# phlash/java-sdr

Hardware: AMD Instinct MI355X
Metric: IQ Msamples/s through FFT+FIR+BPSK demod, 2048-pt frames (higher is better)
Workload: dtype f64

## Files before the change

### java-sdr_amd/binding.py

```python
import ctypes as C
import os
import re

import numpy as np

HERE = os.path.dirname(os.path.abspath(__file__))
ROOT = os.path.dirname(HERE)
_SO = os.environ.get("JSDR_LIB") or os.path.join(HERE, "libjsdr_hip.so")


class JsdrError(RuntimeError):
    pass


def library_path():
    return _SO


def _declared_symbols():
    hdr = open(os.path.join(ROOT, "include", "jsdr_hip.h")).read()
    hdr = re.sub(r"/\*.*?\*/", " ", hdr, flags=re.S)
    return sorted(set(re.findall(r"\b(jsdr_[a-z0-9_]+)\s*\(", hdr)))


# ... 805 lines not shown
                                                        tu if tunings else None, ff, up, C.c_int64(self.max_batch)),
                   "jsdr_bpsk_create_live_channels")
            return
        if do_fft is not None:
            ff = (C.c_int * max(self.nchannels, 1))(*[int(v) for v in do_fft])
            _check(lib().jsdr_bpsk_create_mode_channels(C.byref(self.h), rate, self.samples, ninputs, self.nchannels,
                                                        tu if tunings else None, ff, up, C.c_int64(self.max_batch)),
                   "jsdr_bpsk_create_mode_channels")
            return
        _check(lib().jsdr_bpsk_create_channels(C.byref(self.h), rate, self.samples, ninputs, self.nchannels, tu if tunings else None,
                                               up, C.c_int64(self.max_batch)), "jsdr_bpsk_create_channels")

    def acq_last_launch(self):
        a, b = C.c_int64(), C.c_int64()
        _check(lib().jsdr_bpsk_acq_last_launch(self.h, C.byref(a), C.byref(b)), "jsdr_bpsk_acq_last_launch")
        return a.value, b.value

    def stream(self, inp, ch):
        return inp * self.nchannels + ch

    def channel_info(self):
        a, b = C.c_int(), C.c_int()
        _check(lib().jsdr_bpsk_channel_info(self.h, C.byref(a), C.byref(b)), "jsdr_bpsk_channel_info")
        return a.value, b.value

    def batch_i16(self, raw_dev, input_stride_i16, nsamples, ic=0, qc=0, stream=None):
        super().batch_i16(raw_dev, input_stride_i16, nsamples, ic, qc, stream)

    def batch_f32(self, iq_dev, input_stride_f32, nsamples, stream=None):
        super().batch_f32(iq_dev, input_stride_f32, nsamples, stream)

    def set_channel_tuning(self, channel, tuning_hz):
        _check(lib().jsdr_bpsk_set_channel_tuning(self.h, int(channel), C.c_double(tuning_hz)), "jsdr_bpsk_set_channel_tuning")

    def set_channel_mode(self, channel, do_fft, do_up):
        _check(lib().jsdr_bpsk_set_channel_mode(self.h, int(channel), int(do_fft), int(do_up)), "jsdr_bpsk_set_channel_mode")

    def channel_control(self, channel):
        t, f, u = C.c_double(), C.c_int(), C.c_int()
        _check(lib().jsdr_bpsk_get_channel_control(self.h, int(channel), C.byref(t), C.byref(f), C.byref(u)),
               "jsdr_bpsk_get_channel_control")
        return t.value, f.value, u.value

    def counters(self, inp=0, ch=0):
        return super().counters(self.stream(inp, ch))

    def bits(self, inp=0, ch=0):
        return super().bits(self.stream(inp, ch))

    def fec_results(self, inp=0, ch=0):
        return super().fec_results(self.stream(inp, ch))

    def decoded(self, inp=0, ch=0):
        return super().decoded(self.stream(inp, ch))

    def trace(self, inp=0, ch=0):
        return super().trace(self.stream(inp, ch))

    def state(self, inp=0, ch=0):
        return super().state(self.stream(inp, ch))


class Group:

    def __init__(self, ndev, total_streams, max_batch_samples, devices=None, rate=96000, frame=2048, tuning=12000, do_fft=0,
                 do_up=0, gather_copy=False, with_psd=False):
        self.h = C.c_void_p()
        self.ndev = ndev
        devs = (C.c_int * ndev)(*devices) if devices is not None else None
        flags = (1 if gather_copy else 0) | (2 if with_psd else 0)
        _check(lib().jsdr_group_create(C.byref(self.h), ndev, devs, rate, frame, tuning, do_fft, do_up, total_streams,
                                       C.c_int64(max_batch_samples), flags), "jsdr_group_create")
        n, s, sb, v = C.c_int(), C.c_int(), C.c_int64(), C.c_int()
        _check(lib().jsdr_group_info(self.h, C.byref(n), C.byref(s), C.byref(sb), C.byref(v)), "jsdr_group_info")
        self.streams_per_device, self.slot_bytes, self.rccl_version = s.value, sb.value, v.value
        self.total_streams = total_streams

    def device(self, index):
        d, dem, fft = C.c_int(), C.c_void_p(), C.c_void_p()
        _check(lib().jsdr_group_device(self.h, index, C.byref(d), C.byref(dem), C.byref(fft)), "jsdr_group_device")
        view = Bpsk.__new__(Bpsk)
        view.h, view.nstreams, view.borrowed = dem, self.streams_per_device, True
        return d.value, view

    def batch_i16(self, raw_devs, stride_i16, nsamples, ic=0, qc=0, psd_devs=None):
        raws = (C.c_void_p * self.ndev)(*[_addr(r) for r in raw_devs])
        psds = (C.c_void_p * self.ndev)(*[_addr(p) for p in psd_devs]) if psd_devs is not None else None
        _check(lib().jsdr_group_batch_i16(self.h, raws, C.c_int64(stride_i16), C.c_int64(nsamples), ic, qc, psds),
               "jsdr_group_batch_i16")

    def sync(self):
        _check(lib().jsdr_group_sync(self.h), "jsdr_group_sync")

    def set_tuning(self, tuning_hz):
        _check(lib().jsdr_group_set_tuning(self.h, C.c_double(tuning_hz)), "jsdr_group_set_tuning")

    def set_mode(self, do_fft, do_up):
        _check(lib().jsdr_group_set_mode(self.h, int(do_fft), int(do_up)), "jsdr_group_set_mode")

    def read_slot(self, index, stream):
        out = np.empty(self.slot_bytes, np.uint8)
        _check(lib().jsdr_group_read_slot(self.h, index, stream, _addr(out)), "jsdr_group_read_slot")
        return out

    def gathered(self, index):
        p, nb = C.c_void_p(), C.c_int64()
        self.sync()
        _check(lib().jsdr_group_gathered(self.h, index, C.byref(p), C.byref(nb)), "jsdr_group_gathered")
        dev, _ = self.device(index)
        out = np.empty(nb.value, np.uint8)
        _check(lib().jsdr_set_device(dev), "jsdr_set_device")
        _check(lib().jsdr_memcpy_d2h(_addr(out), p, C.c_size_t(nb.value)), "jsdr_memcpy_d2h")
        return out.reshape(self.total_streams, self.slot_bytes)

    def __del__(self):
        try:
            lib().jsdr_group_destroy(self.h)
        except Exception:
            pass


def unpack_slot(slot, info):
    hdr = np.frombuffer(slot[:64], np.int32)
    nb, nt = int(hdr[0]), int(hdr[1])
    bits = np.frombuffer(slot[info["bits_offset"]:info["bits_offset"] + nb], np.int8)
    fec = []
    for t in range(nt):
        o = info["fec_offset"] + t * 264
        rc, bi = np.frombuffer(slot[o:o + 8], np.int32)
        fec.append((int(rc), int(bi), np.frombuffer(slot[o + 8:o + 264], np.uint8)))
    names = ["nbits", "nfec"] + COUNTER_NAMES[:9]
    return dict(header=dict(zip(names, (int(v) for v in hdr[:11]))), bits=bits, fec=fec)


def demod_scope_layout(n, width):
    out = [np.zeros(max(int(width), 0), np.int32) for _ in range(4)]
    _check(lib().jsdr_demod_scope_layout(int(n), int(width), *[_addr(a) if a.size else None for a in out], int(width)),
           "jsdr_demod_scope_layout")
    return tuple(out)


class Demod:

    def __init__(self, rate=96000, n=2048, nstreams=1, max_batch_samples=None):
        self.rate, self.n, self.S = rate, n, nstreams
        self.max_batch = max_batch_samples or n
        self.h = C.c_void_p()
        _check(lib().jsdr_demod_create(C.byref(self.h), rate, n, nstreams, C.c_int64(self.max_batch)), "jsdr_demod_create")

    def configure(self, mode, dofir=0, dodwn=0, doagc=0):
        _check(lib().jsdr_demod_configure(self.h, mode, dofir, dodwn, doagc), "jsdr_demod_configure")

    def weights(self, flo, fhi):
        w = np.empty(21, np.float32)
        phi = C.c_float()
        _check(lib().jsdr_demod_weights(self.h, flo, fhi, _addr(w), C.byref(phi)), "jsdr_demod_weights")
        return w, np.float32(phi.value)

    def batch_i16(self, raw_dev, stride_i16, nsamples, audio_dev, audio_stride_i16, ic=0, qc=0, stream=None):
        _check(lib().jsdr_demod_batch_i16(self.h, _addr(raw_dev), C.c_int64(stride_i16), C.c_int64(nsamples), ic, qc,
                                          _addr(audio_dev), C.c_int64(audio_stride_i16), C.c_void_p(stream)),
               "jsdr_demod_batch_i16")

    def batch_f32(self, iq_dev, stride_f32, nsamples, audio_dev, audio_stride_i16, stream=None):
        _check(lib().jsdr_demod_batch_f32(self.h, _addr(iq_dev), C.c_int64(stride_f32), C.c_int64(nsamples),
                                          _addr(audio_dev), C.c_int64(audio_stride_i16), C.c_void_p(stream)),
               "jsdr_demod_batch_f32")

    def batch_host_i16(self, raw, nsamples, ic=0, qc=0):
        raw = np.ascontiguousarray(raw, np.int16).reshape(self.S, 2 * nsamples)
        d_in = DeviceBuffer.from_host(raw)
        d_out = DeviceBuffer(raw.nbytes)
        self.batch_i16(d_in, 2 * nsamples, nsamples, d_out, 2 * nsamples, ic, qc)
        return d_out.to_host(np.int16).reshape(self.S, 2 * nsamples)

    def receive(self, buf):
        buf = np.ascontiguousarray(buf, np.float32)
        assert buf.size == 2 * self.n
        out = np.empty(2 * self.n, np.int16)
        _check(lib().jsdr_demod_receive_f32(self.h, _addr(buf), _addr(out)), "jsdr_demod_receive_f32")
        return out

    def frame_stats(self, stream=0):
        mx, av = C.c_float(), C.c_float()
        _check(lib().jsdr_demod_frame_stats(self.h, stream, C.byref(mx), C.byref(av)), "jsdr_demod_frame_stats")
        return np.float32(mx.value), np.float32(av.value)

    def state(self):
        car, phi = C.c_float(), C.c_float()
        _check(lib().jsdr_demod_state(self.h, C.byref(car), C.byref(phi)), "jsdr_demod_state")
        return np.float32(car.value), np.float32(phi.value)

    def scope_i16(self, raw_dev, stride_i16, nsamples, audio_dev, audio_stride_i16, width, height, trace_dev=None, spec_dev=None,
                  dbg_dev=None, ic=0, qc=0, stream=None):
        _check(lib().jsdr_demod_scope_i16(self.h, _addr(raw_dev), C.c_int64(stride_i16), C.c_int64(nsamples), int(ic), int(qc),
                                          _addr(audio_dev), C.c_int64(audio_stride_i16), int(width), int(height), _addr(trace_dev),
                                          _addr(spec_dev), _addr(dbg_dev), C.c_void_p(stream)), "jsdr_demod_scope_i16")

    def scope_f32(self, iq_dev, stride_f32, nsamples, audio_dev, audio_stride_i16, width, height, trace_dev=None, spec_dev=None,
                  dbg_dev=None, stream=None):
        _check(lib().jsdr_demod_scope_f32(self.h, _addr(iq_dev), C.c_int64(stride_f32), C.c_int64(nsamples), _addr(audio_dev),
                                          C.c_int64(audio_stride_i16), int(width), int(height), _addr(trace_dev), _addr(spec_dev),
                                          _addr(dbg_dev), C.c_void_p(stream)), "jsdr_demod_scope_f32")

    def scope_chunk(self, frames):
        _check(lib().jsdr_demod_scope_chunk(self.h, int(frames)), "jsdr_demod_scope_chunk")

    def scope_kernel(self):
        return lib().jsdr_demod_scope_kernel(self.h).decode()

    def profile_enable(self, on):
        _check(lib().jsdr_demod_profile_enable(self.h, int(on)), "jsdr_demod_profile_enable")

    def profile_read(self):
        k = lib().jsdr_demod_profile_count()
        ms = np.zeros(k, np.float64)
        cnt = np.zeros(k, np.int32)
        _check(lib().jsdr_demod_profile_read(self.h, _addr(ms), _addr(cnt)), "jsdr_demod_profile_read")
        return {lib().jsdr_demod_profile_name(i).decode(): (float(ms[i]), int(cnt[i])) for i in range(k)}

    def __del__(self):
        try:
            lib().jsdr_demod_destroy(self.h)
        except Exception:
            pass


class DemodChannels(Demod):

    def __init__(self, rate=96000, n=2048, ninputs=1, nchannels=1, max_batch_samples=None):
        self.rate, self.n, self.ninputs, self.nchannels = rate, n, ninputs, nchannels
        self.S = ninputs * nchannels
        self.max_batch = max_batch_samples or n
        self.h = C.c_void_p()
        _check(lib().jsdr_demod_create_channels(C.byref(self.h), rate, n, ninputs, nchannels, C.c_int64(self.max_batch)),
               "jsdr_demod_create_channels")

    def stream(self, inp, ch):
        return inp * self.nchannels + ch

    def channel_info(self):
        a, b = C.c_int(), C.c_int()
        _check(lib().jsdr_demod_channel_info(self.h, C.byref(a), C.byref(b)), "jsdr_demod_channel_info")
        return a.value, b.value

    def configure_channel(self, channel, mode, dofir=0, dodwn=0, doagc=0):
        _check(lib().jsdr_demod_configure_channel(self.h, int(channel), int(mode), int(dofir), int(dodwn), int(doagc)),
               "jsdr_demod_configure_channel")

    def channel_weights(self, channel, flo, fhi):
        w = np.empty(21, np.float32)
        phi = C.c_float()
        _check(lib().jsdr_demod_channel_weights(self.h, int(channel), int(flo), int(fhi), _addr(w), C.byref(phi)),
               "jsdr_demod_channel_weights")
        return w, np.float32(phi.value)

    def channel_control(self, channel):
        v = [C.c_int() for _ in range(6)]
        _check(lib().jsdr_demod_get_channel(self.h, int(channel), *[C.byref(x) for x in v]), "jsdr_demod_get_channel")
        return tuple(x.value for x in v)

    def channel_state(self, channel):
        car, phi = C.c_float(), C.c_float()
        _check(lib().jsdr_demod_channel_state(self.h, int(channel), C.byref(car), C.byref(phi)), "jsdr_demod_channel_state")
        return np.float32(car.value), np.float32(phi.value)

    def batch_i16(self, raw_dev, input_stride_i16, nsamples, audio_dev, audio_stride_i16, ic=0, qc=0, stream=None):
        super().batch_i16(raw_dev, input_stride_i16, nsamples, audio_dev, audio_stride_i16, ic, qc, stream)

    def batch_f32(self, iq_dev, input_stride_f32, nsamples, audio_dev, audio_stride_i16, stream=None):
        super().batch_f32(iq_dev, input_stride_f32, nsamples, audio_dev, audio_stride_i16, stream)

    def batch_host_i16(self, raw, nsamples, ic=0, qc=0):
        raw = np.ascontiguousarray(raw, np.int16).reshape(self.ninputs, 2 * nsamples)
        d_in = DeviceBuffer.from_host(raw)
        d_out = DeviceBuffer(self.S * 2 * nsamples * 2)
        self.batch_i16(d_in, 2 * nsamples, nsamples, d_out, 2 * nsamples, ic, qc)
        return d_out.to_host(np.int16).reshape(self.ninputs, self.nchannels, 2 * nsamples)

    def receive(self, buf):
        buf = np.ascontiguousarray(buf, np.float32)
        assert buf.size == 2 * self.n
        out = np.empty(self.nchannels * 2 * self.n, np.int16)
        _check(lib().jsdr_demod_receive_f32(self.h, _addr(buf), _addr(out)), "jsdr_demod_receive_f32")
        return out.reshape(self.nchannels, 2 * self.n)


class RecordingInfo(C.Structure):
    _fields_ = [("format", C.c_int), ("encoding", C.c_int), ("channels", C.c_int), ("rate", C.c_int),
                ("bits", C.c_int), ("frames", C.c_int64), ("data_offset", C.c_int64)]


def waterfall_lines(psd, n, width, peak_rgb=0x00FFFF):
    psd = np.ascontiguousarray(psd, np.float32).reshape(-1, n + 2)
    d_in = DeviceBuffer.from_host(psd)
    d_out = DeviceBuffer(4 * psd.shape[0] * width)
    _check(lib().jsdr_waterfall_lines(_addr(d_in), C.c_int64(psd.shape[0]), n, width, C.c_uint32(peak_rgb),
                                      _addr(d_out), None), "jsdr_waterfall_lines")
    return d_out.to_host(np.uint32).reshape(psd.shape[0], width)


def waterfall_lines_dev(psd_dev, nframes, n, width, pix_dev, peak_rgb=0x00FFFF, stream=None):
    _check(lib().jsdr_waterfall_lines(_addr(psd_dev), C.c_int64(nframes), n, width, C.c_uint32(peak_rgb),
                                      _addr(pix_dev), stream), "jsdr_waterfall_lines")


def recording_probe(path, raw_channels=2):
    info = RecordingInfo()
    _check(lib().jsdr_recording_probe(os.fsencode(path), raw_channels, C.byref(info)), "jsdr_recording_probe")
    return info


def recordings_load(paths, channels, rate, first_frame, nframes, raw_dev, stream_stride_i16):
    arr = (C.c_char_p * len(paths))(*[os.fsencode(p) for p in paths])
    got = (C.c_int64 * len(paths))()
    _check(lib().jsdr_recordings_load(arr, len(paths), channels, rate, C.c_int64(first_frame), C.c_int64(nframes),
                                      _addr(raw_dev), C.c_int64(stream_stride_i16), got, None), "jsdr_recordings_load")
    return list(got)


def synth_mix64(z):
    m = 0xFFFFFFFFFFFFFFFF
    z = (z + 0x9E3779B97F4A7C15) & m
    z = ((z ^ (z >> 30)) * 0xBF58476D1CE4E5B9) & m
    z = ((z ^ (z >> 27)) * 0x94D049BB133111EB) & m
    return z ^ (z >> 31)


def synth_carrier_tables(amp):
    a = 2.0 * np.pi * np.arange(1024, dtype=np.float64) / 1024.0
    return np.rint(amp * np.cos(a)).astype(np.int16), np.rint(amp * np.sin(a)).astype(np.int16)


def synth_phase_inc_u32(freq_hz, rate):
    return int(round(freq_hz / rate * 2 ** 32)) & 0xFFFFFFFF


def synth_payloads(seed, stream0, nstreams, nframes, out_dev=None, stream=None):
    own = out_dev is None
    if own:
        out_dev = DeviceBuffer(nstreams * nframes * 256)
    _check(lib().jsdr_synth_payloads(C.c_uint64(seed), stream0, nstreams, nframes, _addr(out_dev), C.c_void_p(stream)),
           "jsdr_synth_payloads")
    return out_dev


def synth_diffsign(sym_dev, nsym, nstreams, dsign_dev, stream=None):
    _check(lib().jsdr_synth_diffsign(_addr(sym_dev), C.c_int64(nsym), nstreams, _addr(dsign_dev), C.c_void_p(stream)),
           "jsdr_synth_diffsign")


def synth_dbpsk(out_dev, stride_i16, nstreams, n0, n, dsign_dev, nsym, sps, phase0, phase_inc, cos_dev, sin_dev,
                noise_gain, keys_dev, stream=None):
    _check(lib().jsdr_synth_dbpsk(_addr(out_dev), C.c_int64(stride_i16), nstreams, C.c_int64(n0), C.c_int64(n),
                                  _addr(dsign_dev), C.c_int64(nsym), sps, C.c_uint32(phase0), C.c_uint32(phase_inc),
                                  _addr(cos_dev), _addr(sin_dev), noise_gain, _addr(keys_dev), C.c_void_p(stream)),
           "jsdr_synth_dbpsk")


def synth_tones(out_dev, frame0, nframes, n, cos_dev, noise_gain, key, stream=None):
    _check(lib().jsdr_synth_tones(_addr(out_dev), C.c_int64(frame0), C.c_int64(nframes), n, _addr(cos_dev), noise_gain,
                                  C.c_uint64(key), C.c_void_p(stream)), "jsdr_synth_tones")
```

### java-sdr_amd/csrc/fft_block_body.h

```cpp
    extern __shared__ __align__(16) unsigned char smem[];
    constexpr int FE = lds_frame_elems(N);
    constexpr int TWN = TWG ? 0 : tw_total(R0, R1, R2, R3);
    float2 *tw_own = reinterpret_cast<float2 *>(smem);
    float2 *bufs = tw_own + TWN;
    float *red_val = reinterpret_cast<float *>(bufs + (size_t)FPB * FE);
    int *red_idx = reinterpret_cast<int *>(red_val + FPB * ((T + 63) / 64));
    const float2 *tw_lds = TWG ? a.tw : tw_own;
#ifdef JSDR_X_WGCLK
    const unsigned long long wgclk0 = __builtin_amdgcn_s_memrealtime();
    unsigned long long wgclk_n = 0;
#endif

    const int tid_b = threadIdx.x;
    if constexpr (!TWG) {
        for (int i = tid_b; i < TWN; i += T * FPB) tw_own[i] = a.tw[i];
        __syncthreads();
    }

    const int fib = tid_b / T;
    const int tid = tid_b - fib * T;
    float2 *buf = bufs + (size_t)fib * FE;
    const long long ngroups = (a.nframes + FPB - 1) / FPB;
    auto frame_of = [&](long long g) {
        long long f = g * FPB + fib;
        return f < a.nframes ? f : a.nframes - 1;
    };
    typename RawPoint<IN>::type raw[R0];
    if ((long long)blockIdx.x < ngroups) fft_fetch<N, T, IN, R0>(a, frame_of(blockIdx.x), tid, raw);
    for (long long g = blockIdx.x; g < ngroups; g += gridDim.x) {
        const long long gn = g + gridDim.x;
        fft_frame<N, T, IN, OUT, R0, R1, R2, R3>(a, frame_of(g), frame_of(gn < ngroups ? gn : g), tid, buf, tw_lds, red_val,
                                                 red_idx, fib, raw);
        __syncthreads();
#ifdef JSDR_X_WGCLK
        wgclk_n++;
#endif
    }
#ifdef JSDR_X_WGCLK
    if (tid_b == 0 && blockIdx.x < WGCLK_WGS) {
        unsigned long long *c = g_fft_wgclk[a.wgclk_slot][blockIdx.x];
        c[0] = wgclk0;
        c[1] = __builtin_amdgcn_s_memrealtime();
        c[2] = wgclk_n;
    }
#endif
```

### java-sdr_amd/csrc/fft_common.h

```cpp
#pragma once
#include "common.h"
#include <type_traits>
#include <utility>
#include <vector>

namespace jsdr {

constexpr double cx_pi = 3.14159265358979323846264338327950288;

constexpr double cx_sin_small(double x)
{
    double x2 = x * x, term = x, sum = x;
    for (int i = 1; i < 12; i++) {
        term *= -x2 / ((2 * i) * (2 * i + 1));
        sum += term;
    }
    return sum;
}
constexpr double cx_cos_small(double x)
{
    double x2 = x * x, term = 1.0, sum = 1.0;
    for (int i = 1; i < 12; i++) {
        term *= -x2 / ((2 * i - 1) * (2 * i));
        sum += term;
    }
    return sum;
}
constexpr double cx_cos_turn(int j, int len)
{
    j %= len;
    if (8 * j <= len) return cx_cos_small(2 * cx_pi * j / len);
    if (8 * j <= 3 * len) return -cx_sin_small(2 * cx_pi * (j - 0.25 * len) / len);
    if (8 * j <= 5 * len) return -cx_cos_small(2 * cx_pi * (j - 0.5 * len) / len);
    if (8 * j <= 7 * len) return cx_sin_small(2 * cx_pi * (j - 0.75 * len) / len);
    return cx_cos_small(2 * cx_pi * (j - len) / len);
}
constexpr double cx_sin_turn(int j, int len) { return cx_cos_turn(4 * j + 3 * len, 4 * len); }

typedef float v2f __attribute__((ext_vector_type(2)));
__device__ __forceinline__ v2f to_v(float2 a) { return (v2f){a.x, a.y}; }
__device__ __forceinline__ float2 from_v(v2f v) { return make_float2(v.x, v.y); }
__device__ __forceinline__ v2f vswap(v2f v) { return __builtin_shufflevector(v, v, 1, 0); }
__device__ __forceinline__ v2f vfma(v2f a, v2f b, v2f c) { return __builtin_elementwise_fma(a, b, c); }

__device__ __forceinline__ float2 cadd(float2 a, float2 b) { return from_v(to_v(a) + to_v(b)); }
__device__ __forceinline__ float2 csub(float2 a, float2 b) { return from_v(to_v(a) - to_v(b)); }
__device__ __forceinline__ float2 cmul2(float2 a, float2 w, float2 wq)
{
    const v2f va = to_v(a);
    return from_v(vfma(__builtin_shufflevector(va, va, 1, 1), to_v(wq), __builtin_shufflevector(va, va, 0, 0) * to_v(w)));
}
__device__ __forceinline__ float2 cquad(float2 w) { return from_v(vswap(to_v(w)) * (v2f){-1.0f, 1.0f}); }
__device__ __forceinline__ float2 cmul(float2 a, float2 w) { return cmul2(a, w, cquad(w)); }

template <int LEN, int J>
__device__ __forceinline__ float2 mul_w(float2 d)
{
    const v2f vd = to_v(d);
    if constexpr (J == 0) {
        return d;
    } else if constexpr (4 * J == LEN) {
        return from_v(vswap(vd) * (v2f){1.0f, -1.0f});
    } else if constexpr (8 * J == LEN) {
        constexpr float c = (float)0.70710678118654752440;
        return from_v(vfma(vswap(vd), (v2f){c, -c}, vd * c));
    } else if constexpr (8 * J == 3 * LEN) {
        constexpr float c = (float)0.70710678118654752440;
        return from_v(vfma(vswap(vd), (v2f){c, -c}, vd * -c));
    } else {
        constexpr float c = (float)cx_cos_turn(J, LEN);
        constexpr float s = (float)cx_sin_turn(J, LEN);
        return from_v(vfma(vswap(vd), (v2f){s, -s}, vd * c));
    }
}

template <int LEN, int BASE, int J>
__device__ __forceinline__ void bfly(float2 *x)
{
    constexpr int H = LEN / 2;
    float2 a = x[BASE + J], b = x[BASE + J + H];
    x[BASE + J] = cadd(a, b);
    x[BASE + J + H] = mul_w<LEN, J>(csub(a, b));
}
template <int LEN, int BASE, int... Js>
__device__ __forceinline__ void bfly_group(float2 *x, std::integer_sequence<int, Js...>)
{
    (bfly<LEN, BASE, Js>(x), ...);
}
template <int R, int LEN, int... Bs>
__device__ __forceinline__ void bfly_stage(float2 *x, std::integer_sequence<int, Bs...>)
{
    (bfly_group<LEN, Bs * LEN>(x, std::make_integer_sequence<int, LEN / 2>{}), ...);
}
template <int R, int LEN = R>
__device__ __forceinline__ void dft_reg(float2 *x)
{
    if constexpr (LEN >= 2) {
        bfly_stage<R, LEN>(x, std::make_integer_sequence<int, R / LEN>{});
        dft_reg<R, LEN / 2>(x);
    }
}
constexpr int cx_bitrev(int v, int r)
{
    int o = 0;
    for (int b = 1; b < r; b <<= 1) {
        o = (o << 1) | (v & 1);
        v >>= 1;
    }
    return o;
}

__device__ __forceinline__ int lds_pad(int idx) { return idx + (idx >> 4); }
constexpr int lds_frame_elems(int n) { return n + (n >> 4) + 1; }


enum { IN_I16 = 0, IN_F32 = 1 };
enum { OUT_PSD = 0, OUT_SPEC = 1, OUT_PIX = 2 };

struct FftArgs {
    const void *in;
    float *out;
    const float2 *tw;
    long long nframes;
    int rate;
    int ic, qc;
    int split = 0;
#ifdef JSDR_X_WGCLK
    int wgclk_slot = 0;
#endif
};

struct StreamGeom {
    long long fps;
    long long f0;
    long long in_stride;
    long long out_stride;
    long long out_base;
    long long step_j;
    long long step_in, step_out;
    long long wrap_in, wrap_out;
    long long last_in, last_out;
    int n;
};
template <class BASE>
struct Strided : BASE {
    StreamGeom g;
};
template <class ARGS>
struct is_strided : std::false_type {};
template <class B>
struct is_strided<Strided<B>> : std::true_type {};
inline StreamGeom stream_geom(int n, long long fps, long long in_stride, long long out_stride, long long f0, long long nf, long long out_base)
{
    StreamGeom g = {};
    g.fps = fps;
    g.f0 = f0;
    g.in_stride = in_stride;
    g.out_stride = out_stride;
    g.out_base = out_base;
    g.wrap_in = in_stride - fps * n;
    g.wrap_out = out_stride - fps * (n + 2);
    const long long s = (f0 + nf - 1) / fps, j = (f0 + nf - 1) % fps;
    g.last_in = s * in_stride + j * n;
    g.last_out = out_base + s * out_stride + j * (n + 2);
    g.n = n;
    return g;
}
inline void stream_geom_step(StreamGeom &g, long long step)
{
    const long long ss = step / g.fps;
    g.step_j = step % g.fps;
    g.step_in = ss * g.in_stride + g.step_j * g.n;
    g.step_out = ss * g.out_stride + g.step_j * (g.n + 2);
}
struct FramePos {
    long long f;
    long long j;
    long long in, out;
};
__device__ __forceinline__ FramePos stream_pos(const StreamGeom &g, long long f)
{
    FramePos p;
    const unsigned long long G = (unsigned long long)(g.f0 + f), s = G / (unsigned long long)g.fps;
    p.f = f;
    p.j = (long long)(G - s * (unsigned long long)g.fps);
    p.in = (long long)s * g.in_stride + p.j * g.n;
    p.out = g.out_base + (long long)s * g.out_stride + p.j * (g.n + 2);
    return p;
}
__device__ __forceinline__ void stream_step(const StreamGeom &g, FramePos &p, long long step)
{
    p.f += step;
    p.j += g.step_j;
    p.in += g.step_in;
    p.out += g.step_out;
    if (p.j >= g.fps) {
        p.j -= g.fps;
        p.in += g.wrap_in;
        p.out += g.wrap_out;
    }
}

__device__ __forceinline__ long long frame_first(const FftArgs &, long long f) { return f; }
__device__ __forceinline__ bool frame_more(const FftArgs &a, long long f) { return f < a.nframes; }
__device__ __forceinline__ void frame_next(const FftArgs &, long long &f, long long step) { f += step; }
template <class B>
__device__ __forceinline__ FramePos frame_first(const Strided<B> &a, long long f) { return stream_pos(a.g, f); }
template <class B>
__device__ __forceinline__ bool frame_more(const Strided<B> &a, const FramePos &p) { return p.f < a.nframes; }
template <class B>
__device__ __forceinline__ void frame_next(const Strided<B> &a, FramePos &p, long long step) { stream_step(a.g, p, step); }
__device__ __forceinline__ long long frame_in(long long f, int n) { return f * n; }
__device__ __forceinline__ long long frame_in(const FramePos &p, int) { return p.in; }
__device__ __forceinline__ long long frame_out(long long f, int row) { return f * row; }
__device__ __forceinline__ long long frame_out(const FramePos &p, int) { return p.out; }
__device__ __forceinline__ long long frame_row(long long f) { return f; }
__device__ __forceinline__ long long frame_row(const FramePos &p) { return p.f; }

struct Best {
    float v;
    int k;
};

struct MixedPlan {
    int n = 0, nrad = 0, radix[6] = {1, 1, 1, 1, 1, 1};
    int threads = 0;
    size_t lds_bytes = 0;
    int tw_count = 0;
    bool split2 = false;
    int half_tw_count = 0;
};
bool mixed_plan(int n, MixedPlan &p);
void mixed_twiddles(const MixedPlan &p, float2 *out);
int mixed_launch(const MixedPlan &p, const FftArgs &a, int in_kind, int out_kind, int grid, hipStream_t st);
int mixed_launch_split2(const MixedPlan &p, const FftArgs &a, int in_kind, int out_kind, int num_cu, hipStream_t st);

bool rt_supported(int n);
void rt_twiddles(int n, std::vector<float2> &w);
int rt_launch(const FftArgs &a, int n, int in_kind, int out_kind, int num_cu, hipStream_t st);

bool dft_any_supported(int n);
int dft_any_launch(const FftArgs &a, int n, int in_kind, int out_kind, int num_cu, hipStream_t st);

int mixed_launch_streams(const MixedPlan &p, const Strided<FftArgs> &a, int in_kind, int grid, hipStream_t st);
int mixed_launch_split2_streams(const MixedPlan &p, const Strided<FftArgs> &a, int in_kind, int num_cu, hipStream_t st);
int rt_launch_streams(const Strided<FftArgs> &a, int n, int in_kind, int num_cu, hipStream_t st);
int dft_any_launch_streams(const Strided<FftArgs> &a, int n, int in_kind, int num_cu, hipStream_t st);

}
```

### java-sdr_amd/csrc/fft_psd.hip

```cpp
#include "fft_common.h"
#include "waterfall_dev.h"
#include <math.h>
#include <stdlib.h>
#include <vector>

namespace jsdr {

constexpr bool tw_direct(int P, int R) { return P * R <= 512; }
constexpr int tw_size(int P, int R) { return P <= 1 ? 0 : (tw_direct(P, R) ? 2 * P * (R - 1) : P); }
constexpr int tw_total(int R0, int R1, int R2, int R3)
{
    return tw_size(R0, R1) + (R2 > 1 ? tw_size(R0 * R1, R2) : 0) + (R3 > 1 ? tw_size(R0 * R1 * R2, R3) : 0);
}

constexpr int ilog2_c(int n) { return n <= 1 ? 0 : 1 + ilog2_c(n / 2); }

template <int R, int P>
__device__ __forceinline__ void apply_twiddles(float2 *v, int k, const float2 *tab)
{
    if constexpr (P > 1) {
        if constexpr (tw_direct(P, R)) {
#pragma unroll
            for (int r = 1; r < R; r++) {
                const float4 t = reinterpret_cast<const float4 *>(tab)[(r - 1) * P + k];
                v[r] = cmul2(v[r], make_float2(t.x, t.y), make_float2(t.z, t.w));
            }
        } else {
            float2 w1 = tab[k];
            float2 w[R], wq[R];
            w[1] = w1;
            wq[1] = cquad(w1);
#pragma unroll
            for (int r = 2; r < R; r++) {
                w[r] = (r & 1) ? cmul2(w[r - 1], w1, wq[1]) : cmul2(w[r / 2], w[r / 2], wq[r / 2]);
                wq[r] = cquad(w[r]);
            }
#pragma unroll
            for (int r = 1; r < R; r++) v[r] = cmul2(v[r], w[r], wq[r]);
        }
    }
}

template <int R, int... Rs>
__device__ __forceinline__ void store_lds(float2 *dst, const float2 *v, int j0, int p, std::integer_sequence<int, Rs...>)
{
    ((dst[lds_pad(j0 + Rs * p)] = v[cx_bitrev(Rs, R)]), ...);
}

template <int IN>
struct RawPoint {
    using type = int;
};
template <>
struct RawPoint<IN_F32> {
    using type = float2;
};
template <int N, int T, int IN, int R, class FR>
__device__ __forceinline__ void fft_fetch(const FftArgs &a, FR frame, int tid, typename RawPoint<IN>::type (&w)[R])
{
    constexpr int NB = N / R;
    static_assert(NB == T, "one first-pass butterfly per thread");
    const typename RawPoint<IN>::type *src = reinterpret_cast<const typename RawPoint<IN>::type *>(a.in) +
#ifdef JSDR_X_FFT_SMALLSET
        (frame_row(frame) & 8191) * N;
#else
        frame_in(frame, N);
#endif
#pragma unroll
    for (int r = 0; r < R; r++) {
#ifdef JSDR_X_FFT_NOLOAD
        if constexpr (IN == IN_I16) w[r] = (tid + r * NB) * 2654435761u + (int)(size_t)src;
        else w[r] = make_float2((float)(tid + r), (float)(size_t)src);
#else
        w[r] = src[tid + r * NB];
#endif
    }
}

enum { SC_NONE = 0, SC_IN = 1, SC_OUT = 2 };

struct FftPixArgs : FftArgs {
    unsigned *pix;
    float *maxo;
    float *peak;
    int width;
    unsigned peak_rgb;
};

template <int N>
__device__ __forceinline__ float psd_db(float2 x)
{
    constexpr float L2 = 3.0102999566398120f;
    constexpr float OFF = 3.0102999566398120f * (2.0f - 2.0f * (float)ilog2_c(N));
    return L2 * __log2f(x.x * x.x + x.y * x.y) + OFF;
}

__device__ __forceinline__ int row_pad(int idx) { return idx + (idx >> 5); }
constexpr bool fft_i16_scaled(int R0, int R1) { return tw_direct(R0, R1); }

template <int N, int T, int IN, int OUT, int R, int P, bool FIRST, bool LAST, class RAW = int, int SC = SC_NONE, class FR>
__device__ __forceinline__ void fft_pass(const FftArgs &a, FR frame, bool active, int tid, float2 *buf,
                                         const float2 *tab, Best &best, const RAW *raw = nullptr)
{
    constexpr int NB = N / R;
    static_assert(NB % T == 0, "butterflies per pass must be a multiple of the threads per frame");
    constexpr int ITERS = NB / T;
    constexpr bool TO_LDS = !LAST || OUT == OUT_PIX;
    constexpr int GROUP = TO_LDS ? ITERS : 1;
#pragma unroll
    for (int g0 = 0; g0 < ITERS; g0 += GROUP) {
        float2 v[GROUP][R];
#pragma unroll
        for (int gi = 0; gi < GROUP; gi++) {
            const int b = (g0 + gi) * T + tid;
            if constexpr (FIRST) {
                if (active) {
                    if constexpr (IN == IN_I16) {
                        const RAW *w = raw;
                        auto cvt = [](int s) { return SC == SC_IN ? i16_to_float_java_2p15(s) : i16_to_float_java(s); };
                        if ((a.ic | a.qc) == 0) {
#pragma unroll
                            for (int r = 0; r < R; r++)
                                v[gi][r] = make_float2(cvt((int)(short)(w[r] & 0xffff)), cvt(w[r] >> 16));
                        } else {
#pragma unroll
                            for (int r = 0; r < R; r++) {
                                int si = java_short_add((int)(short)(w[r] & 0xffff), a.ic);
                                int sq = java_short_add(w[r] >> 16, a.qc);
                                v[gi][r] = make_float2(cvt(si), cvt(sq));
                            }
                        }
                    } else {
#pragma unroll
                        for (int r = 0; r < R; r++) v[gi][r] = raw[r];
                    }
                } else {
#pragma unroll
                    for (int r = 0; r < R; r++) v[gi][r] = make_float2(0.f, 0.f);
                }
            } else {
#pragma unroll
                for (int r = 0; r < R; r++) v[gi][r] = buf[lds_pad(b + r * NB)];
            }
            if constexpr (SC == SC_OUT) v[gi][0] = from_v(to_v(v[gi][0]) * I16_2P15_UNSCALE);
            apply_twiddles<R, P>(v[gi], b & (P - 1), tab);
            dft_reg<R>(v[gi]);
        }
        if constexpr (!FIRST && TO_LDS) __syncthreads();
#pragma unroll
        for (int gi = 0; gi < GROUP; gi++) {
            const int b = (g0 + gi) * T + tid;
            const int k = b & (P - 1);
            const int j0 = (b - k) * R + k;
            if constexpr (!LAST) {
                store_lds<R>(buf, v[gi], j0, P, std::make_integer_sequence<int, R>{});
            } else if (active) {
                if constexpr (OUT == OUT_SPEC) {
                    float2 *dst = reinterpret_cast<float2 *>(a.out) + frame_out(frame, N);
#pragma unroll
                    for (int r = 0; r < R; r++) dst[j0 + r * P] = v[gi][cx_bitrev(r, R)];
                } else {
                    float *dst = a.out + frame_out(frame, N + 2);
                    float db[R];
#pragma unroll
                    for (int r = 0; r < R; r++) {
                        db[r] = psd_db<N>(v[gi][cx_bitrev(r, R)]);
                        if constexpr (OUT == OUT_PIX) {
                            reinterpret_cast<float *>(buf)[row_pad(j0 + r * P)] = db[r];
                        } else {
#ifndef JSDR_X_FFT_NOSTORE
                            dst[j0 + r * P] = db[r];
#endif
                        }
                    }
                    float gm = db[0];
#pragma unroll
                    for (int r = 1; r < R; r++) gm = fmaxf(gm, db[r]);
                    int gk = 0x7fffffff;
#pragma unroll
                    for (int r = R - 1; r >= 0; r--) gk = (db[r] == gm) ? j0 + r * P : gk;
                    const bool take = (gm > best.v) | ((gm == best.v) & (gk < best.k));
                    best.v = take ? gm : best.v;
                    best.k = take ? gk : best.k;
                }
            }
        }
    }
    if constexpr (!LAST) __syncthreads();
}

template <int N, int T, int IN, int OUT, int R0, int R1, int R2, int R3, class ARGS, class FR, class FN>
__device__ __forceinline__ void fft_frame(const ARGS &a, FR frame, FN next, int tid, float2 *buf,
                                          const float2 *tw_lds, float *red_val, int *red_idx, int frame_in_block,
                                          typename RawPoint<IN>::type (&raw)[R0])
{
    using RAW = typename RawPoint<IN>::type;
    constexpr bool active = true;
    constexpr int NPASS = (R1 == 1) ? 1 : (R2 == 1) ? 2 : (R3 == 1) ? 3 : 4;
    static_assert(NPASS >= 2, "the first pass must not be the last");
    static_assert(R0 * R1 * R2 * R3 == N, "radix plan must multiply to N");
    Best best;
    best.v = -3.402823466e+38f;
    best.k = 0x7fffffff;
    constexpr int O1 = 0, O2 = tw_size(R0, R1), O3 = O2 + tw_size(R0 * R1, R2);
    constexpr bool SC = IN == IN_I16 && fft_i16_scaled(R0, R1);
    fft_pass<N, T, IN, OUT, R0, 1, true, false, RAW, SC ? SC_IN : SC_NONE>(a, frame, active, tid, buf, tw_lds, best, raw);
    auto prefetch = [&] { fft_fetch<N, T, IN, R0>(a, next, tid, raw); };
    if constexpr (NPASS == 2) prefetch();
    fft_pass<N, T, IN, OUT, R1, R0, false, NPASS == 2, int, SC ? SC_OUT : SC_NONE>(a, frame, active, tid, buf, tw_lds + O1, best);
    if constexpr (NPASS >= 3) {
        if constexpr (NPASS == 3) prefetch();
        fft_pass<N, T, IN, OUT, R2, R0 * R1, false, NPASS == 3>(a, frame, active, tid, buf, tw_lds + O2, best);
    }
    if constexpr (NPASS >= 4) {
        prefetch();
        fft_pass<N, T, IN, OUT, R3, R0 * R1 * R2, false, NPASS == 4>(a, frame, active, tid, buf, tw_lds + O3, best);
    }

    [[maybe_unused]] const float *row = reinterpret_cast<const float *>(buf);
    static_assert(N + (N >> 5) + 1 <= 2 * lds_frame_elems(N), "the padded row fits the image");

    if constexpr (OUT == OUT_PSD || OUT == OUT_PIX) {
        float bestv = best.v;
        int bestk = best.k;
        constexpr int W = (T < 64) ? T : 64;
#pragma unroll
        for (int off = W / 2; off >= 1; off >>= 1) {
            float ov = __shfl_xor(bestv, off, W);
            int ok = __shfl_xor(bestk, off, W);
            const bool take = (ov > bestv) | ((ov == bestv) & (ok < bestk));
            bestv = take ? ov : bestv;
            bestk = take ? ok : bestk;
        }
        if constexpr (T > 64) {
            constexpr int NW = T / 64;
            int fb = frame_in_block, wv = tid >> 6;
            if constexpr (OUT == OUT_PIX) {
                fb = __builtin_amdgcn_readfirstlane(fb);
                wv = __builtin_amdgcn_readfirstlane(wv);
            }
            if ((tid & 63) == 0) {
                red_val[fb * NW + wv] = bestv;
                red_idx[fb * NW + wv] = bestk;
            }
            __syncthreads();
            if (tid == 0) {
                for (int w = 1; w < NW; w++) {
                    float ov = red_val[fb * NW + w];
                    int ok = red_idx[fb * NW + w];
                    if (ov > bestv || (ov == bestv && ok < bestk)) {
                        bestv = ov;
                        bestk = ok;
                    }
                }
            }
        }
        if (tid == 0 && active) {
            int p = (bestv > -3.402823466e+38f) ? 2 * bestk : -1;
            float m = (p >= 0) ? bestv : -3.402823466e+38f;
            const int datlen = 2 * N;
            if (p >= datlen / 2) p -= datlen;
            int hz = (int)((unsigned)p * (unsigned)a.rate) / datlen;
            if constexpr (OUT == OUT_PIX) {
                if (a.peak) {
                    a.peak[frame_row(frame) * 2] = (float)hz;
                    a.peak[frame_row(frame) * 2 + 1] = m;
                }
            } else {
                float *dst = a.out + frame_out(frame, N + 2);
                dst[N] = (float)hz;
                dst[N + 1] = m;
            }
        }
    }

    if constexpr (OUT == OUT_PIX) {
        if constexpr (T <= 64) __syncthreads();
        const int width = a.width, half = width / 2;
        const float step = wf_step(N, width);
        const int l = java_f2i(step);
        const WfColour colour = wf_colour(a.peak_rgb);
        unsigned *prow = a.pix + frame_row(frame) * width;
        float *mrow = a.maxo ? a.maxo + frame_row(frame) * width : nullptr;
        for (int p = tid; p < width; p += T) {
            const float r = wf_getmax([&](int i) { return row[row_pad(i)]; }, java_f2i((float)p * step), l);
            if (mrow) mrow[p] = r;
            const int q = p + half;
            prow[q >= width ? q - width : q] = wf_pixel(r, colour);
        }
    }
}

#ifdef JSDR_X_WGCLK
constexpr int WGCLK_SLOTS = 128, WGCLK_WGS = 1024;
__device__ unsigned long long g_fft_wgclk[WGCLK_SLOTS][WGCLK_WGS][3];
#endif

template <int N, int T, int FPB, int IN, int OUT, int R0, int R1, int R2, int R3, bool TWG = false>
__global__ __launch_bounds__(T *FPB, (N == 2048 ? 4 : 1)) void k_fft(FftArgs a)
{
#include "fft_block_body.h"
}

template <int N, int T, int FPB, int IN, int R0, int R1, int R2, int R3>
__global__ __launch_bounds__(T *FPB, (N == 2048 ? 4 : N == 8192 ? 3 : 1)) void k_fft_pix(FftPixArgs a)
{
    constexpr int OUT = OUT_PIX;
    constexpr bool TWG = false;
#include "fft_block_body.h"
}

struct LdsFrame {
    const long long *slot;
    long long f;
};
struct LdsNext {
    long long *slot;
    const StreamGeom *g;
    long long step;
    bool more, past;
};
__device__ __forceinline__ long long frame_out(const LdsFrame &p, int) { return p.slot[3]; }
__device__ __forceinline__ long long frame_row(const LdsFrame &p) { return p.f; }
__device__ __forceinline__ long long frame_in(const LdsNext &q, int)
{
    if (!q.more) return q.slot[1];
    FramePos p;
    p.f = 0;
    p.j = q.slot[0];
    p.in = q.slot[1];
    p.out = q.slot[2];
    stream_step(*q.g, p, q.step);
    if (q.past) {
        p.in = q.g->last_in;
        p.out = q.g->last_out;
    }
    q.slot[0] = p.j;
    q.slot[1] = p.in;
    q.slot[2] = p.out;
    return p.in;
}

template <int N, int T, int FPB, int IN, int OUT, int R0, int R1, int R2, int R3, class ARGS>
__global__ __launch_bounds__(T *FPB, (N == 2048 ? 4 : (N == 8192 && OUT == OUT_PIX) ? 3 : N == 64 ? 8 : (N == 4096 && OUT == OUT_PSD) ? 4 : (N == 128 && OUT == OUT_PIX && IN == IN_F32) ? 6 : 1)) void k_fft_streams(ARGS a)
{
    extern __shared__ __align__(16) unsigned char smem[];
    constexpr int FE = lds_frame_elems(N);
    constexpr int TWN = tw_total(R0, R1, R2, R3);
    float2 *tw_own = reinterpret_cast<float2 *>(smem);
    float2 *bufs = tw_own + TWN;
    float *red_val = reinterpret_cast<float *>(bufs + (size_t)FPB * FE);
    int *red_idx = reinterpret_cast<int *>(red_val + FPB * ((T + 63) / 64));
    [[maybe_unused]] long long *slots = reinterpret_cast<long long *>(red_idx + FPB * ((T + 63) / 64));

    const int tid_b = threadIdx.x;
    for (int i = tid_b; i < TWN; i += T * FPB) tw_own[i] = a.tw[i];
    __syncthreads();

    int fib = FPB == 1 ? 0 : tid_b / T;
    const int tid = tid_b - fib * T;
    if constexpr (T >= 64 && FPB > 1) fib = __builtin_amdgcn_readfirstlane(fib);
    float2 *buf = bufs + (size_t)fib * FE;
    const long long ngroups = (a.nframes + FPB - 1) / FPB;
    const long long step = (long long)gridDim.x * FPB;
    if ((long long)blockIdx.x >= ngroups) return;
    auto clamped = [&](FramePos p) {
        if (p.f >= a.nframes) {
            p.f = a.nframes - 1;
            p.in = a.g.last_in;
            p.out = a.g.last_out;
        }
        return p;
    };
    typename RawPoint<IN>::type raw[R0];
    if constexpr (T >= 64) {
        FramePos walk = stream_pos(a.g, (long long)blockIdx.x * FPB + fib);
        FramePos cur = clamped(walk);
        fft_fetch<N, T, IN, R0>(a, cur, tid, raw);
        for (long long g = blockIdx.x; g < ngroups; g += gridDim.x) {
            FramePos next = cur;
            if (g + gridDim.x < ngroups) {
                stream_step(a.g, walk, step);
                next = clamped(walk);
            }
            fft_frame<N, T, IN, OUT, R0, R1, R2, R3>(a, cur, next, tid, buf, tw_own, red_val, red_idx, fib, raw);
            __syncthreads();
            cur = next;
        }
    } else {
        long long *slot = slots + 4 * fib;
        {
            const FramePos first = clamped(stream_pos(a.g, (long long)blockIdx.x * FPB + fib));
            slot[0] = first.j;
            slot[1] = first.in;
            slot[2] = first.out;
            fft_fetch<N, T, IN, R0>(a, first, tid, raw);
        }
        for (long long g = blockIdx.x; g < ngroups; g += gridDim.x) {
            slot[3] = slot[2];
            const long long f = g * FPB + fib, fn = f + step;
            const LdsFrame cur = {slot, f < a.nframes ? f : a.nframes - 1};
            const LdsNext next = {slot, &a.g, step, g + gridDim.x < ngroups, fn >= a.nframes};
            fft_frame<N, T, IN, OUT, R0, R1, R2, R3>(a, cur, next, tid, buf, tw_own, red_val, red_idx, fib, raw);
            __syncthreads();
        }
    }
}

template <int N, int FPB, int T, int R0, int R1, int R2, int R3, bool TWG = false>
constexpr size_t fft_lds_bytes()
{
    return sizeof(float2) * ((TWG ? (size_t)0 : (size_t)tw_total(R0, R1, R2, R3)) + (size_t)FPB * lds_frame_elems(N)) +
           (sizeof(float) + sizeof(int)) * FPB * ((T + 63) / 64);
}

struct Launcher {
    void (*launch)(const FftArgs &, int grid, hipStream_t) = nullptr;
    void (*launch_pix)(const FftPixArgs &, int grid, hipStream_t) = nullptr;
    void (*launch_s)(const Strided<FftArgs> &, int grid, hipStream_t) = nullptr;
    void (*launch_pix_s)(const Strided<FftPixArgs> &, int grid, hipStream_t) = nullptr;
    int frames_per_block = 0;
    size_t lds_bytes = 0;
    int block = 0;
    int radix[4] = {1, 1, 1, 1};
};

template <int N, int T, int FPB, int IN, int OUT, int R0, int R1, int R2, int R3, bool TWG = false>
static void launch_impl(const FftArgs &a, int grid, hipStream_t s)
{
    constexpr size_t lds = fft_lds_bytes<N, FPB, T, R0, R1, R2, R3, TWG>();
    hipLaunchKernelGGL((k_fft<N, T, FPB, IN, OUT, R0, R1, R2, R3, TWG>), dim3(grid), dim3(T * FPB), lds, s, a);
}

template <int N, int T, int FPB, int IN, int R0, int R1, int R2, int R3>
static void launch_pix_impl(const FftPixArgs &a, int grid, hipStream_t s)
{
    constexpr size_t lds = fft_lds_bytes<N, FPB, T, R0, R1, R2, R3, false>();
    hipLaunchKernelGGL((k_fft_pix<N, T, FPB, IN, R0, R1, R2, R3>), dim3(grid), dim3(T * FPB), lds, s, a);
}

template <int N, int T, int FPB, int IN, int OUT, int R0, int R1, int R2, int R3, class ARGS>
static void launch_streams_impl(const ARGS &a, int grid, hipStream_t s)
{
    constexpr size_t lds = fft_lds_bytes<N, FPB, T, R0, R1, R2, R3, false>() + (T < 64 ? sizeof(long long) * 4 * FPB : 0);
    hipLaunchKernelGGL((k_fft_streams<N, T, FPB, IN, OUT, R0, R1, R2, R3, ARGS>), dim3(grid), dim3(T * FPB), lds, s, a);
}

template <int N, int T, int FPB, int R0, int R1, int R2, int R3, bool TWG = false>
static Launcher make_launcher(int in, int out)
{
    Launcher l;
    l.frames_per_block = FPB;
    l.block = T * FPB;
    l.lds_bytes = fft_lds_bytes<N, FPB, T, R0, R1, R2, R3, TWG>();
    l.radix[0] = R0;
    l.radix[1] = R1;
    l.radix[2] = R2;
    l.radix[3] = R3;
    if (in == IN_I16 && out == OUT_PSD) l.launch = launch_impl<N, T, FPB, IN_I16, OUT_PSD, R0, R1, R2, R3, TWG>;
    if (in == IN_F32 && out == OUT_PSD) l.launch = launch_impl<N, T, FPB, IN_F32, OUT_PSD, R0, R1, R2, R3, TWG>;
    if (in == IN_F32 && out == OUT_SPEC) l.launch = launch_impl<N, T, FPB, IN_F32, OUT_SPEC, R0, R1, R2, R3, TWG>;
    if constexpr (!TWG) {
        if (in == IN_I16 && out == OUT_PIX) l.launch_pix = launch_pix_impl<N, T, FPB, IN_I16, R0, R1, R2, R3>;
        if (in == IN_F32 && out == OUT_PIX) l.launch_pix = launch_pix_impl<N, T, FPB, IN_F32, R0, R1, R2, R3>;
        if (in == IN_I16 && out == OUT_PSD) l.launch_s = launch_streams_impl<N, T, FPB, IN_I16, OUT_PSD, R0, R1, R2, R3, Strided<FftArgs>>;
        if (in == IN_F32 && out == OUT_PSD) l.launch_s = launch_streams_impl<N, T, FPB, IN_F32, OUT_PSD, R0, R1, R2, R3, Strided<FftArgs>>;
        if (in == IN_I16 && out == OUT_PIX) l.launch_pix_s = launch_streams_impl<N, T, FPB, IN_I16, OUT_PIX, R0, R1, R2, R3, Strided<FftPixArgs>>;
        if (in == IN_F32 && out == OUT_PIX) l.launch_pix_s = launch_streams_impl<N, T, FPB, IN_F32, OUT_PIX, R0, R1, R2, R3, Strided<FftPixArgs>>;
    }
    return l;
}

static Launcher pick_launcher(int n, int in, int out)
{
    switch (n) {
        case 64: return make_launcher<64, 8, 32, 8, 8, 1, 1>(in, out);
        case 128: return make_launcher<128, 8, 32, 16, 8, 1, 1>(in, out);
        case 256: return make_launcher<256, 16, 16, 16, 16, 1, 1>(in, out);
        case 512: return make_launcher<512, 64, 4, 8, 8, 8, 1>(in, out);
        case 1024: return make_launcher<1024, 64, 4, 16, 8, 8, 1>(in, out);
        case 2048: return make_launcher<2048, 128, 2, 16, 16, 8, 1>(in, out);
        case 4096: return make_launcher<4096, 256, 1, 16, 16, 16, 1>(in, out);
        case 8192: return make_launcher<8192, 512, 1, 16, 16, 8, 4>(in, out);
        default: return Launcher();
    }
}

__global__ __launch_bounds__(256) void k_waterfall_aux(const float *__restrict__ psd, long long nframes, int n, int width,
                                                       float *__restrict__ maxo, float *__restrict__ peak)
{
    const float step = wf_step(n, width);
    const int l = java_f2i(step);
    for (long long frame = blockIdx.x; frame < nframes; frame += gridDim.x) {
        const float *a = psd + frame * (n + 2);
        if (maxo)
            for (int p = threadIdx.x; p < width; p += 256)
                maxo[frame * width + p] = wf_getmax([&](int i) { return a[i]; }, java_f2i((float)p * step), l);
        if (peak && threadIdx.x < 2) peak[frame * 2 + threadIdx.x] = a[n + threadIdx.x];
    }
}

}

using namespace jsdr;

struct jsdr_fft {
    int n = 0;
    int rate = 0;
    DevBuf<float2> tw;
    DevBuf<float2> tw_i16;
    DevBuf<unsigned char> in_stage;
    DevBuf<float> out_stage;
    PinnedStage pin;
    bool pin_lazy_done = false;
    int num_cu = 256;
    bool mixed = false;
    MixedPlan mplan;
    bool rt = false;
    bool direct = false;
    long long last_items = 0, last_grid = 0;
    int share_wgs_per_cu = 0;
    DevBuf<float> wf_rows;
    std::string wf_kernel;
};
constexpr long long WF_CHUNK = 1024;

#ifdef JSDR_X_WGCLK
static long long g_wgclk_log[WGCLK_SLOTS][3];
static void fft_wgclk_report()
{
    const char *path = getenv("JSDR_X_WGCLK_OUT");
    FILE *f = fopen(path ? path : "wgclk_fft.csv", "w");
    static unsigned long long cc[WGCLK_SLOTS][WGCLK_WGS][3];
    if (f && hipMemcpyFromSymbol(cc, HIP_SYMBOL(g_fft_wgclk), sizeof(cc)) == hipSuccess) {
        fprintf(f, "launch,items,grid,ticket,wg,t0,t1,n\n");
// ... 495 lines not shown
```

Before: 258,200.

## Use buffer-resource loads/stores and DPP wave reductions for wave-multiple FFT frames

For thread counts that are multiples of the wavefront size, frame input loads and spectrum/PSD output stores now go through raw buffer resource intrinsics with a per-lane offset and a constant offset, instead of flat global pointers. The peak-bin argmax reduction replaces the shuffle-xor loop with DPP-based integer max/min reductions on an order-preserving float key. The frame index is also made wave-uniform via readfirstlane. These aim to cut address arithmetic, VGPR use and cross-lane shuffle cost. In exchange they rely on buffer bounds semantics and a two-pass reduction that must preserve tie-breaking. A binding stream argument cast is also fixed.

Result: faster. 263,800 (median of 6 runs) (+2.2%).

```diff
diff --git a/java-sdr_amd/binding.py b/java-sdr_amd/binding.py
--- a/java-sdr_amd/binding.py
+++ b/java-sdr_amd/binding.py
@@ -1131,7 +1131,7 @@
 
 def waterfall_lines_dev(psd_dev, nframes, n, width, pix_dev, peak_rgb=0x00FFFF, stream=None):
     _check(lib().jsdr_waterfall_lines(_addr(psd_dev), C.c_int64(nframes), n, width, C.c_uint32(peak_rgb),
-                                      _addr(pix_dev), stream), "jsdr_waterfall_lines")
+                                      _addr(pix_dev), C.c_void_p(stream)), "jsdr_waterfall_lines")
 
 
 def recording_probe(path, raw_channels=2):
diff --git a/java-sdr_amd/csrc/fft_block_body.h b/java-sdr_amd/csrc/fft_block_body.h
--- a/java-sdr_amd/csrc/fft_block_body.h
+++ b/java-sdr_amd/csrc/fft_block_body.h
@@ -17,8 +17,9 @@
         __syncthreads();
     }
 
-    const int fib = tid_b / T;
+    int fib = tid_b / T;
     const int tid = tid_b - fib * T;
+    if constexpr (frame_is_waves(T)) fib = FPB == 1 ? 0 : __builtin_amdgcn_readfirstlane(fib);
     float2 *buf = bufs + (size_t)fib * FE;
     const long long ngroups = (a.nframes + FPB - 1) / FPB;
     auto frame_of = [&](long long g) {
diff --git a/java-sdr_amd/csrc/fft_common.h b/java-sdr_amd/csrc/fft_common.h
--- a/java-sdr_amd/csrc/fft_common.h
+++ b/java-sdr_amd/csrc/fft_common.h
@@ -222,6 +222,57 @@
     int k;
 };
 
+constexpr bool frame_is_waves(int T) { return T % 64 == 0; }
+
+using WaveRow = __amdgpu_buffer_rsrc_t;
+__device__ __forceinline__ WaveRow wave_row(const void *base, unsigned bytes)
+{
+    return __builtin_amdgcn_make_buffer_rsrc(const_cast<void *>(base), 0, (int)bytes, 0x00020000);
+}
+template <class V>
+__device__ __forceinline__ V wave_row_load(WaveRow row, unsigned lane_bytes, unsigned const_bytes)
+{
+    static_assert(sizeof(V) == 4 || sizeof(V) == 8, "one or two dwords a lane");
+    if constexpr (sizeof(V) == 4) return __builtin_bit_cast(V, __builtin_amdgcn_raw_buffer_load_b32(row, lane_bytes, const_bytes, 0));
+    else return __builtin_bit_cast(V, __builtin_amdgcn_raw_buffer_load_b64(row, lane_bytes, const_bytes, 0));
+}
+template <class V>
+__device__ __forceinline__ void wave_row_store(WaveRow row, unsigned lane_bytes, unsigned const_bytes, V v)
+{
+    static_assert(sizeof(V) == 4 || sizeof(V) == 8, "one or two dwords a lane");
+    if constexpr (sizeof(V) == 4)
+        __builtin_amdgcn_raw_buffer_store_b32(__builtin_bit_cast(unsigned, v), row, lane_bytes, const_bytes, 0);
+    else
+        __builtin_amdgcn_raw_buffer_store_b64(__builtin_bit_cast(decltype(__builtin_amdgcn_raw_buffer_load_b64(row, 0, 0, 0)), v), row,
+                                              lane_bytes, const_bytes, 0);
+}
+
+template <int CTRL>
+__device__ __forceinline__ int dpp_i32(int x)
+{
+    return __builtin_amdgcn_update_dpp(0, x, CTRL, 0xf, 0xf, true);
+}
+constexpr int DPP_QUAD_1032 = 0xB1, DPP_QUAD_2301 = 0x4E, DPP_ROW_HALF_MIRROR = 0x141, DPP_ROW_MIRROR = 0x140;
+template <bool MAX, int CTRL>
+__device__ __forceinline__ int pick_dpp(int x)
+{
+    const int o = dpp_i32<CTRL>(x);
+    return MAX ? (o > x ? o : x) : (o < x ? o : x);
+}
+template <bool MAX>
+__device__ __forceinline__ int wave_reduce_i32(int x)
+{
+    x = pick_dpp<MAX, DPP_QUAD_1032>(x);
+    x = pick_dpp<MAX, DPP_QUAD_2301>(x);
+    x = pick_dpp<MAX, DPP_ROW_HALF_MIRROR>(x);
+    x = pick_dpp<MAX, DPP_ROW_MIRROR>(x);
+    const int r0 = __builtin_amdgcn_readlane(x, 0), r1 = __builtin_amdgcn_readlane(x, 16);
+    const int r2 = __builtin_amdgcn_readlane(x, 32), r3 = __builtin_amdgcn_readlane(x, 48);
+    const int a = MAX ? (r0 > r1 ? r0 : r1) : (r0 < r1 ? r0 : r1), b = MAX ? (r2 > r3 ? r2 : r3) : (r2 < r3 ? r2 : r3);
+    return MAX ? (a > b ? a : b) : (a < b ? a : b);
+}
+__device__ __forceinline__ int f32_order_key(int bits) { return bits ^ (int)((unsigned)(bits >> 31) >> 1); }
+
 struct MixedPlan {
     int n = 0, nrad = 0, radix[6] = {1, 1, 1, 1, 1, 1};
     int threads = 0;
diff --git a/java-sdr_amd/csrc/fft_psd.hip b/java-sdr_amd/csrc/fft_psd.hip
--- a/java-sdr_amd/csrc/fft_psd.hip
+++ b/java-sdr_amd/csrc/fft_psd.hip
@@ -66,13 +66,16 @@
 #else
         frame_in(frame, N);
 #endif
+    using RAW = typename RawPoint<IN>::type;
+    [[maybe_unused]] const WaveRow row = wave_row(src, N * (unsigned)sizeof(RAW));
 #pragma unroll
     for (int r = 0; r < R; r++) {
 #ifdef JSDR_X_FFT_NOLOAD
         if constexpr (IN == IN_I16) w[r] = (tid + r * NB) * 2654435761u + (int)(size_t)src;
         else w[r] = make_float2((float)(tid + r), (float)(size_t)src);
 #else
-        w[r] = src[tid + r * NB];
+        if constexpr (frame_is_waves(T)) w[r] = wave_row_load<RAW>(row, tid * (unsigned)sizeof(RAW), r * NB * (unsigned)sizeof(RAW));
+        else w[r] = src[tid + r * NB];
 #endif
     }
 }
@@ -158,7 +161,12 @@
                 if constexpr (OUT == OUT_SPEC) {
                     float2 *dst = reinterpret_cast<float2 *>(a.out) + frame_out(frame, N);
 #pragma unroll
-                    for (int r = 0; r < R; r++) dst[j0 + r * P] = v[gi][cx_bitrev(r, R)];
+                    for (int r = 0; r < R; r++) {
+                        if constexpr (frame_is_waves(T))
+                            wave_row_store(wave_row(dst, N * 8u), j0 * 8u, r * P * 8u, v[gi][cx_bitrev(r, R)]);
+                        else
+                            dst[j0 + r * P] = v[gi][cx_bitrev(r, R)];
+                    }
                 } else {
                     float *dst = a.out + frame_out(frame, N + 2);
                     float db[R];
@@ -169,7 +177,8 @@
                             reinterpret_cast<float *>(buf)[row_pad(j0 + r * P)] = db[r];
                         } else {
 #ifndef JSDR_X_FFT_NOSTORE
-                            dst[j0 + r * P] = db[r];
+                            if constexpr (frame_is_waves(T)) wave_row_store(wave_row(dst, (N + 2) * 4u), j0 * 4u, r * P * 4u, db[r]);
+                            else dst[j0 + r * P] = db[r];
 #endif
                         }
                     }
@@ -224,13 +233,20 @@
         float bestv = best.v;
         int bestk = best.k;
         constexpr int W = (T < 64) ? T : 64;
-#pragma unroll
-        for (int off = W / 2; off >= 1; off >>= 1) {
-            float ov = __shfl_xor(bestv, off, W);
-            int ok = __shfl_xor(bestk, off, W);
-            const bool take = (ov > bestv) | ((ov == bestv) & (ok < bestk));
-            bestv = take ? ov : bestv;
-            bestk = take ? ok : bestk;
+        if constexpr (frame_is_waves(T)) {
+            const int key = f32_order_key(__builtin_bit_cast(int, bestv));
+            const int mkey = wave_reduce_i32<true>(key);
+            bestk = wave_reduce_i32<false>(key == mkey ? bestk : 0x7fffffff);
+            bestv = __builtin_bit_cast(float, f32_order_key(mkey));
+        } else {
+#pragma unroll
+            for (int off = W / 2; off >= 1; off >>= 1) {
+                float ov = __shfl_xor(bestv, off, W);
+                int ok = __shfl_xor(bestk, off, W);
+                const bool take = (ov > bestv) | ((ov == bestv) & (ok < bestk));
+                bestv = take ? ov : bestv;
+                bestk = take ? ok : bestk;
+            }
         }
         if constexpr (T > 64) {
             constexpr int NW = T / 64;
```
